# sdwyc/ROLO

Hardware: AMD Instinct MI355X
Metric: scans/sec (128k-pt frame, 20 GN iters) (higher is better)
Workload: dtype f64

## Files before the change

### rolo_amd/csrc/knn_cov.hip

```cpp
#include <cstdio>
#include <cstring>
#include <string.h>
#include "rolo_internal.hpp"
#include "dev_math.hpp"
#include "voxel_dev.hpp"
#ifdef ROLO_KNN_ROCPRIM_SORT
#include <rocprim/rocprim.hpp>
#endif
#include <cfloat>
#include <climits>

namespace rolo {

namespace {


constexpr int BBOX_BLOCKS = 128;
constexpr int BBOX_PART = 16;

__global__ __launch_bounds__(256) void bbox_kernel(KnnPair A, int* bbox) {
  __shared__ float smn[4][3], smx[4][3];
  const int which = blockIdx.x / BBOX_BLOCKS, blk = blockIdx.x - which * BBOX_BLOCKS;
  const float4* __restrict__ p = A.c[which].xyz;
  const int n = A.c[which].n;
// ... 477 lines not shown
#pragma unroll
    for (int i = 0; i < 9; i++) Ci[i] /= nrm;
    inv3(Ci, out);
  } else {
    const double A[9] = {cxx, cxy, cxz, cxy, cyy, cyz, cxz, cyz, czz};
    double U[9], V[9], sv[3];
    jacobi_svd3(A, U, sv, V);
    double v0 = 1, v1 = 1, v2 = 1e-3;
    if (reg == ROLO_REG_MIN_EIG) { v0 = fmax(sv[0], 1e-3); v1 = fmax(sv[1], 1e-3); v2 = fmax(sv[2], 1e-3); }
    else if (reg == ROLO_REG_NORMALIZED_MIN_EIG) { double m = fmax(sv[0], fmax(sv[1], sv[2])); v0 = fmax(sv[0] / m, 1e-3); v1 = fmax(sv[1] / m, 1e-3); v2 = fmax(sv[2] / m, 1e-3); }
    else if (reg == ROLO_REG_PLANE_S) { double s = sv[0] + sv[1] + sv[2]; v0 = sv[0] / s; v1 = sv[1] / s; v2 = 1e-3; }
#pragma unroll
    for (int a = 0; a < 3; a++)
#pragma unroll
      for (int b = 0; b < 3; b++) out[a * 3 + b] = (U[a * 3 + 0] * v0) * V[b * 3 + 0] + (U[a * 3 + 1] * v1) * V[b * 3 + 1] + (U[a * 3 + 2] * v2) * V[b * 3 + 2];
    if (nrm && reg == ROLO_REG_PLANE) {
      const double s3 = U[0 * 3 + 2] * V[0 * 3 + 2] + U[1 * 3 + 2] * V[1 * 3 + 2] + U[2 * 3 + 2] * V[2 * 3 + 2];
      const double al = sqrt(1.0 - (s3 < 0 ? -1e-3 : 1e-3));
      const double s1 = U[0 * 3 + 0] * V[0 * 3 + 0] + U[1 * 3 + 0] * V[1 * 3 + 0] + U[2 * 3 + 0] * V[2 * 3 + 0];
      const double s2 = U[0 * 3 + 1] * V[0 * 3 + 1] + U[1 * 3 + 1] * V[1 * 3 + 1] + U[2 * 3 + 1] * V[2 * 3 + 1];
      const bool plane_form = s1 > 0 && s2 > 0;
      const size_t pn = (size_t)n;
      nrm[qi] = plane_form ? al * V[0 * 3 + 2] : __builtin_nan(""); nrm[pn + qi] = al * V[1 * 3 + 2]; nrm[2 * pn + qi] = al * V[2 * 3 + 2];
    }
  }
  const size_t pitch = (size_t)n;
  c6[0] = out[0]; c6[1] = 0.5 * (out[1] + out[3]); c6[2] = 0.5 * (out[2] + out[6]); c6[3] = out[4]; c6[4] = 0.5 * (out[5] + out[7]); c6[5] = out[8];
#pragma unroll
  for (int d = 0; d < 6; d++) cov[d * pitch + qi] = c6[d];
}

template <int KMAX>
ROLO_DEV void knn_neighbourhood_moments(const int (&ki)[KMAX], int kk, const float4* __restrict__ orig, double (&m6)[6]) {
  float px[KMAX], py[KMAX], pz[KMAX];
#pragma unroll
  for (int u = 0; u < KMAX; u++) {
    const float4 p = (u < kk) ? orig[ki[u]] : make_float4(0.f, 0.f, 0.f, 0.f);
    px[u] = p.x; py[u] = p.y; pz[u] = p.z;
  }
  double mx = 0, my = 0, mz = 0;
#pragma unroll
  for (int u = 0; u < KMAX; u++) if (u < kk) { mx += (double)px[u]; my += (double)py[u]; mz += (double)pz[u]; }
  mx /= kk; my /= kk; mz /= kk;
  double cxx = 0, cxy = 0, cxz = 0, cyy = 0, cyz = 0, czz = 0;
#pragma unroll
  for (int u = 0; u < KMAX; u++) if (u < kk) {
    const double ax = (double)px[u] - mx, ay = (double)py[u] - my, az = (double)pz[u] - mz;
    cxx += ax * ax; cxy += ax * ay; cxz += ax * az; cyy += ay * ay; cyz += ay * az; czz += az * az;
  }
  m6[0] = cxx / kk; m6[1] = cxy / kk; m6[2] = cxz / kk; m6[3] = cyy / kk; m6[4] = cyz / kk; m6[5] = czz / kk;
}

template <int KMAX>
ROLO_DEV void knn_covariance_tail(const int (&ki)[KMAX], int kk, const float4* __restrict__ orig, int n, int qi, int reg,
                                  double* __restrict__ cov, double (&c6)[6], double* __restrict__ nrm = nullptr) {
  double m6[6];
  knn_neighbourhood_moments<KMAX>(ki, kk, orig, m6);
  knn_covariance_finish(m6[0], m6[1], m6[2], m6[3], m6[4], m6[5], n, qi, reg, cov, c6, nrm);
}

ROLO_DEV void knn_covariance_tail_loop(const int32_t* __restrict__ nbr, size_t n_sorted, int j, int kk, const float4* __restrict__ orig, int n, int qi, int reg,
                                       double* __restrict__ cov, double (&c6)[6], double* __restrict__ nrm = nullptr) {
  double mx = 0, my = 0, mz = 0;
  for (int u = 0; u < kk; u++) { const float4 p = orig[nbr[(size_t)u * n_sorted + j]]; mx += (double)p.x; my += (double)p.y; mz += (double)p.z; }
  mx /= kk; my /= kk; mz /= kk;
  double cxx = 0, cxy = 0, cxz = 0, cyy = 0, cyz = 0, czz = 0;
  for (int u = 0; u < kk; u++) {
    const float4 p = orig[nbr[(size_t)u * n_sorted + j]];
    const double ax = (double)p.x - mx, ay = (double)p.y - my, az = (double)p.z - mz;
    cxx += ax * ax; cxy += ax * ay; cxz += ax * az; cyy += ay * ay; cyz += ay * az; czz += az * az;
  }
  cxx /= kk; cxy /= kk; cxz /= kk; cyy /= kk; cyz /= kk; czz /= kk;
  knn_covariance_finish(cxx, cxy, cxz, cyy, cyz, czz, n, qi, reg, cov, c6, nrm);
}
}
}

#include "knn_walk.hpp"

namespace rolo {

bool knn_voxel_fuse_supported() {
#ifdef ROLO_KNN_ROCPRIM_SORT
  return false;
#else
  return true;
#endif
}

size_t knn_bbox_ints() { return BBOX_PART + 2 * BBOX_BLOCKS * 6; }

size_t knn_sort_temp_bytes(int n) {
#ifdef ROLO_KNN_ROCPRIM_SORT
  size_t bytes = 0;
  (void)rocprim::radix_sort_pairs(nullptr, bytes, (uint32_t*)nullptr, (uint32_t*)nullptr, (uint32_t*)nullptr, (uint32_t*)nullptr,
                                  (size_t)n, 0, 31, (hipStream_t)0);
  return bytes;
#else
  (void)n;
  return sizeof(int) * SORT_PASSES * SORT_NB * SORT_D;
#endif
}

hipError_t launch_knn_build(const KnnPair& A_in, void* sort_tmp, size_t sort_tmp_bytes, uint32_t* keys0, uint32_t* keys1,
                            uint32_t* vals0, uint32_t* vals1, int* bbox, const VoxelFuse& vf, hipStream_t s) {
  KnnPair A = A_in;
  bool have_parts = true;
  for (int i = 0; i < A.n_clouds; i++) have_parts = have_parts && A.c[i].bpart != nullptr && A.c[i].n_bpart > 0;
  if (!have_parts) for (int i = 0; i < A.n_clouds; i++) { A.c[i].bpart = bbox + BBOX_PART + i * BBOX_BLOCKS * 6; A.c[i].n_bpart = BBOX_BLOCKS; }
  const int nc = A.n_clouds;
  const int n_total = A.c[0].n + (nc > 1 ? A.c[1].n : 0);
#ifdef ROLO_KNN_ROCPRIM_SORT
  const int tile_ = ((n_total + SORT_NB - 1) / SORT_NB + SORT_T - 1) / SORT_T * SORT_T;
  if (!have_parts) bbox_kernel<<<BBOX_BLOCKS * nc, 256, 0, s>>>(A, bbox);
  morton_kernel<<<SORT_NB + (vf.enabled ? VF_CLEAR_BLOCKS : 0), SORT_T, 0, s>>>(A, bbox, keys0, vals0, n_total, tile_, nullptr, vf);
  hipError_t e = rocprim::radix_sort_pairs(sort_tmp, sort_tmp_bytes, keys0, keys1, vals0, vals1, (size_t)n_total, 0, nc > 1 ? KEY_BITS : KEY_BITS - 1, s);
  if (e != hipSuccess) return e;
  const uint32_t* order = vals1;
#else
  (void)sort_tmp_bytes;
  int* cnt = static_cast<int*>(sort_tmp);
  const int gvf = vf.enabled ? ((vf.n_tgt + SORT_PASSES - 1) / SORT_PASSES + SORT_T - 1) / SORT_T : 0;
  const int tile = ((n_total + SORT_NB - 1) / SORT_NB + SORT_T - 1) / SORT_T * SORT_T;
  if (!have_parts) bbox_kernel<<<BBOX_BLOCKS * nc, 256, 0, s>>>(A, bbox);
  morton_kernel<<<SORT_NB + (vf.enabled ? VF_CLEAR_BLOCKS : 0), SORT_T, 0, s>>>(A, bbox, keys0, vals0, n_total, tile, cnt, vf);
  uint32_t *ki = keys0, *vi = vals0, *ko = keys1, *vo = vals1;
  for (int p = 0; p < SORT_PASSES; p++) {
    if (p > 0) sort_hist_kernel<<<SORT_NB, SORT_T, 0, s>>>(ki, n_total, tile, p, cnt);
    sort_scatter_kernel<<<SORT_NB + gvf, SORT_T, 0, s>>>(ki, vi, ko, vo, n_total, tile, p, cnt, vf);
    uint32_t* t1 = ki; ki = ko; ko = t1; t1 = vi; vi = vo; vo = t1;
  }
  const uint32_t* order = vi;
#endif
  static_assert(256 % KNN_LEAF == 0 && (KNN_LEAF & (KNN_LEAF - 1)) == 0, "leaf_kernel reduces a leaf inside a wavefront");
  const int l0 = (A.c[0].P * KNN_LEAF + 255) / 256, l1 = nc > 1 ? (A.c[1].P * KNN_LEAF + 255) / 256 : 0;
  leaf_kernel<<<l0 + l1, 256, 0, s>>>(A, l0, order);
  constexpr int LPB = 256 / KNN_LEAF;
  int count0 = A.c[0].P >= LPB ? A.c[0].P / LPB : A.c[0].P, count1 = nc > 1 ? (A.c[1].P >= LPB ? A.c[1].P / LPB : A.c[1].P) : 1;
  while (count0 > 1 || count1 > 1) {
    const int chunk0 = count0 < 512 ? count0 : 512, chunk1 = count1 < 512 ? count1 : 512;
    const int b0 = count0 > 1 ? count0 / chunk0 : 0, b1 = count1 > 1 ? count1 / chunk1 : 0;
    tree_reduce_kernel<<<b0 + b1, 256, 0, s>>>(A.c[0].boxes, count0, chunk0, b0, nc > 1 ? A.c[1].boxes : nullptr, count1, chunk1);
    if (count0 > 1) count0 /= chunk0;
    if (count1 > 1) count1 /= chunk1;
  }
  return hipGetLastError();
}

#ifdef ROLO_KNN_STATS
extern "C" int rolo_debug_wave_records(unsigned* out ) {
  (void)hipDeviceSynchronize();
  return hipMemcpyFromSymbol(out, HIP_SYMBOL(g_knn_wave_rec), sizeof(unsigned) * 16384 * 8) == hipSuccess ? 0 : -1;
}
#endif

static inline int slice_blocks(const KnnCloud& c) { return (c.q_end - c.q_begin + 255) / 256; }

constexpr int KNN_SUB_MAX_PACKETS = 1792;
hipError_t launch_knn_walk(const KnnPair& A, int k, int regularization_or_minus1, const VoxelFuse& vf, hipStream_t s, int coop_budget, int* lanes_out, bool device_busy, bool moments) {
  if (lanes_out) *lanes_out = 1;
  constexpr int QPB = 256;
  const int n0 = A.c[0].q_end - A.c[0].q_begin, n1 = A.n_clouds > 1 ? A.c[1].q_end - A.c[1].q_begin : 0;
  const int g0 = (n0 + QPB - 1) / QPB, g1 = (n1 + QPB - 1) / QPB;
  if (g0 + g1 == 0) return hipSuccess;
  (void)vf;
  constexpr int pad = 0;
  if (k > 64) {
    if (regularization_or_minus1 >= 0) return hipErrorInvalidValue;
    KnnPair R = A;
    for (int r = 0; 64 * r < k; r++) {
      const int kr = k - 64 * r < 64 ? k - 64 * r : 64;
      for (int i = 0; i < R.n_clouds; i++) { R.c[i].slot0 = 64 * r; R.c[i].k_total = k; }
      if (r == 0) knn_walk_kernel<64, false><<<g0 + g1, 256, pad, s>>>(R, g0, kr, -1);
      else knn_walk_kernel<64, false, true><<<g0 + g1, 256, pad, s>>>(R, g0, kr, -1);
    }
    return hipGetLastError();
  }
  if (k == 20) {
    if (regularization_or_minus1 >= 0) knn_walk_kernel<20, true><<<g0 + g1, 256, pad, s>>>(A, g0, k, regularization_or_minus1);
    else if (coop_budget > 0) {
      const int packets = (n0 + 63) / 64 + (n1 + 63) / 64;
      static const int force_nw = [] {
        const char* e = getenv("ROLO_KNN_COOP_NW");
        if (!e) return 0;
        const int v = atoi(e);
        if (v == 4 || v == 8 || v == 16) return v;
        fprintf(stderr, "librolo_hip: ROLO_KNN_COOP_NW=%s is not one of 4 / 8 / 16: ignored\n", e);
        return 0;
      }();
      const int nw = force_nw ? force_nw : (packets >= 16 * 256 ? 16 : (packets >= 8 * 256 ? 8 : 4));
      const int G4 = g0 + g1, G = (G4 + nw / 4 - 1) / (nw / 4);
      if (nw == 16) knn_walk_coop_kernel<16><<<G, 1024, 0, s>>>(A, g0, G4, coop_budget);
      else if (nw == 8) knn_walk_coop_kernel<8><<<G, 512, 0, s>>>(A, g0, G4, coop_budget);
      else knn_walk_coop_kernel<4><<<G, 256, 0, s>>>(A, g0, G4, coop_budget);
    }
    else {
      static const int sub_env = [] {
        const char* e = getenv("ROLO_KNN_SUB");
        if (!e) return -1;
        const int v = atoi(e);
        if (v == 0 || v == 1 || v == 2 || v == 4) return v;
        fprintf(stderr, "librolo_hip: ROLO_KNN_SUB=%s is not one of 0 / 1 / 2 / 4: ignored (the walk is picked by size)\n", e);
        return -1;
      }();
      const int packets = (n0 + 63) / 64 + (n1 + 63) / 64;
      const int lanes = sub_env < 0 ? (packets <= KNN_SUB_MAX_PACKETS ? 4 : (device_busy ? 0 : 2)) : (sub_env == 2 ? 2 : (sub_env ? 4 : 0));
      if (lanes_out) *lanes_out = lanes ? lanes : 1;
      static const int walk_pad = [] {
        const char* e = getenv("ROLO_KNN_WALK_WGS"); const int v = e ? atoi(e) : 0;
        const int pad_bytes = (v >= 1 && v <= 8) ? (160 * 1024 / v - 1024 - 512) & ~255 : 0;
        if (pad_bytes > 48 * 1024) {
          bool ok = hipFuncSetAttribute(reinterpret_cast<const void*>(&knn_walk_kernel<20, false>), hipFuncAttributeMaxDynamicSharedMemorySize, pad_bytes) == hipSuccess;
          ok = ok && hipFuncSetAttribute(reinterpret_cast<const void*>(&knn_walk_sub_kernel<2>), hipFuncAttributeMaxDynamicSharedMemorySize, pad_bytes) == hipSuccess;
          ok = ok && hipFuncSetAttribute(reinterpret_cast<const void*>(&knn_walk_sub_kernel<4>), hipFuncAttributeMaxDynamicSharedMemorySize, pad_bytes) == hipSuccess;
          if (!ok) { (void)hipGetLastError(); fprintf(stderr, "librolo_hip: ROLO_KNN_WALK_WGS=%d needs %d bytes of dynamic LDS, which this runtime refuses: ignored\n", v, pad_bytes); return 0; }
        }
        return pad_bytes;
      }();
      if (lanes == 4) { const int s0 = (n0 + 63) / 64, s1 = (n1 + 63) / 64; if (moments) knn_walk_sub_kernel<4, true><<<s0 + s1, 256, walk_pad, s>>>(A, s0); else knn_walk_sub_kernel<4><<<s0 + s1, 256, walk_pad, s>>>(A, s0); }
      else if (lanes == 2) { const int s0 = (n0 + 127) / 128, s1 = (n1 + 127) / 128; if (moments) knn_walk_sub_kernel<2, true><<<s0 + s1, 256, walk_pad, s>>>(A, s0); else knn_walk_sub_kernel<2><<<s0 + s1, 256, walk_pad, s>>>(A, s0); }
      else if (moments) knn_walk_kernel<20, false, false, true><<<g0 + g1, 256, walk_pad, s>>>(A, g0, k, -1);
      else knn_walk_kernel<20, false><<<g0 + g1, 256, walk_pad, s>>>(A, g0, k, -1);
    }
  }
  else {
    if (k > 32) {
      if (regularization_or_minus1 >= 0) knn_walk_kernel<64, true><<<g0 + g1, 256, pad, s>>>(A, g0, k, regularization_or_minus1);
      else knn_walk_kernel<64, false><<<g0 + g1, 256, pad, s>>>(A, g0, k, -1);
    } else if (regularization_or_minus1 >= 0) knn_walk_kernel<32, true><<<g0 + g1, 256, pad, s>>>(A, g0, k, regularization_or_minus1);
    else knn_walk_kernel<32, false><<<g0 + g1, 256, pad, s>>>(A, g0, k, -1);
  }
  return hipGetLastError();
}

hipError_t launch_knn_unstage(const KnnPair& A, bool own_slice_only, const VoxelFuse& vf, hipStream_t s) {
  const int g0 = own_slice_only ? slice_blocks(A.c[0]) : (A.c[0].n_sorted + 255) / 256;
  const int g1 = A.n_clouds > 1 ? (own_slice_only ? slice_blocks(A.c[1]) : (A.c[1].n_sorted + 255) / 256) : 0;
  if (g0 + g1 == 0) return hipSuccess;
  VoxelFuse v = vf;
  if (own_slice_only) v.enabled = 0;
  knn_unstage_kernel<<<g0 + g1, 256, 0, s>>>(A, g0, own_slice_only ? 1 : 0, v);
  return hipGetLastError();
}

hipError_t launch_knn_tail(const KnnPair& A, int k, int regularization, const VoxelFuse& vf, hipStream_t s, bool moments) {
  const int g0 = slice_blocks(A.c[0]), g1 = A.n_clouds > 1 ? slice_blocks(A.c[1]) : 0;
  if (g0 + g1 == 0) return hipSuccess;
  if (k > 64) knn_tail_loop_kernel<<<g0 + g1, 256, 0, s>>>(A, g0, k, regularization, vf);
  else if (k == 20 && moments) knn_tail_kernel<20, true><<<g0 + g1, 256, 0, s>>>(A, g0, k, regularization, vf);
  else if (k == 20) knn_tail_kernel<20><<<g0 + g1, 256, 0, s>>>(A, g0, k, regularization, vf);
  else if (k <= 32) knn_tail_kernel<32><<<g0 + g1, 256, 0, s>>>(A, g0, k, regularization, vf);
  else knn_tail_kernel<64><<<g0 + g1, 256, 0, s>>>(A, g0, k, regularization, vf);
  return hipGetLastError();
}

}
```

### rolo_amd/csrc/knn_packet.hpp

```cpp
#pragma once
#include "rolo_internal.hpp"
#include "dev_math.hpp"
#include <cfloat>
#include <climits>

#ifndef KNN_STAT
#ifdef ROLO_KNN_STATS
#define KNN_STAT(x) x
#else
#define KNN_STAT(x)
#endif
#endif

namespace rolo {
namespace {

constexpr int WALK_STACK = KNN_WALK_STACK;

ROLO_DEV float box_d2(const float4& lo, const float4& hi, const float4& q) {
  float dx = fmaxf(fmaxf(__fsub_rn(lo.x, q.x), __fsub_rn(q.x, hi.x)), 0.f);
  float dy = fmaxf(fmaxf(__fsub_rn(lo.y, q.y), __fsub_rn(q.y, hi.y)), 0.f);
  float dz = fmaxf(fmaxf(__fsub_rn(lo.z, q.z), __fsub_rn(q.z, hi.z)), 0.f);
  return __fadd_rn(__fadd_rn(__fmul_rn(dx, dx), __fmul_rn(dy, dy)), __fmul_rn(dz, dz));
}

ROLO_DEV double key_pack(float d2, int idx) {
  return __longlong_as_double((long long)(((unsigned long long)__float_as_uint(d2) << 32) | (unsigned)idx));
}
ROLO_DEV float key_d2(double k) { return __uint_as_float((unsigned)((unsigned long long)__double_as_longlong(k) >> 32)); }
ROLO_DEV int key_idx(double k) { return (int)(unsigned)((unsigned long long)__double_as_longlong(k) & 0xffffffffull); }

ROLO_DEV double vmin_f64(double a, double b) { double r; asm("v_min_f64 %0, %1, %2" : "=v"(r) : "v"(a), "v"(b)); return r; }
ROLO_DEV double vmax_f64(double a, double b) { double r; asm("v_max_f64 %0, %1, %2" : "=v"(r) : "v"(a), "v"(b)); return r; }
#ifndef ROLO_KNN_SPLIT_MINMAX
ROLO_DEV void insert_slot(double& ks, double ksm1, double c) { asm("v_min_f64 %0, %1, %0\n\tv_max_f64 %0, %2, %0" : "+&v"(ks) : "v"(c), "v"(ksm1)); }
#else
ROLO_DEV void insert_slot(double& ks, double ksm1, double c) { ks = vmax_f64(ksm1, vmin_f64(c, ks)); }
#endif
#ifndef ROLO_KNN_B1
#define ROLO_KNN_B1 15
#define ROLO_KNN_B2 10
#define ROLO_KNN_B3 5
#endif
template <int KMAX>
ROLO_DEV void insert_tiered(double (&K)[KMAX], double ck) {
  constexpr int B1 = KMAX == 20 ? ROLO_KNN_B1 : 3 * (KMAX / 4), B2 = KMAX == 20 ? ROLO_KNN_B2 : 2 * (KMAX / 4), B3 = KMAX == 20 ? ROLO_KNN_B3 : KMAX / 4;
#pragma unroll
  for (int s = KMAX - 1; s >= B1; s--) insert_slot(K[s], K[s - 1], ck);
  if (__any(ck < K[B1 - 1])) {
#pragma unroll
    for (int s = B1 - 1; s >= B2; s--) insert_slot(K[s], K[s - 1], ck);
    if (__any(ck < K[B2 - 1])) {
#pragma unroll
      for (int s = B2 - 1; s >= B3; s--) insert_slot(K[s], K[s - 1], ck);
      if (__any(ck < K[B3 - 1])) {
#pragma unroll
        for (int s = B3 - 1; s >= 1; s--) insert_slot(K[s], K[s - 1], ck);
        K[0] = vmin_f64(ck, K[0]);
      }
    }
  }
}

typedef float sgpr16 __attribute__((ext_vector_type(16)));
#ifndef ROLO_KNN_ASM_LOADS
#define ROLO_KNN_ASM_LOADS 0
#endif
constexpr bool KNN_PLAIN_ASM = ROLO_KNN_ASM_LOADS != 0;
ROLO_DEV const float4* uniform_ptr(const float4* p) {
  const unsigned long long v = (unsigned long long)p;
  const unsigned lo = (unsigned)__builtin_amdgcn_readfirstlane((int)(unsigned)v), hi = (unsigned)__builtin_amdgcn_readfirstlane((int)(unsigned)(v >> 32));
  return (const float4*)(((unsigned long long)hi << 32) | lo);
}
template <bool ASM>
ROLO_DEV void sload_leaf(const float4* __restrict__ p_, float4 (&pts)[KNN_LEAF]) {
  if (!ASM) {
#pragma unroll
    for (int u = 0; u < KNN_LEAF; u++) pts[u] = p_[u];
    return;
  }
  const float4* p = uniform_ptr(p_);
#if 1
  static_assert(KNN_LEAF == 16 || KNN_LEAF == 8, "leaf size");
  sgpr16 a, b;
  if (KNN_LEAF == 16) {
    sgpr16 c, d;
    asm("s_load_dwordx16 %0, %4, 0x0\n\ts_load_dwordx16 %1, %4, 0x40\n\ts_load_dwordx16 %2, %4, 0x80\n\ts_load_dwordx16 %3, %4, 0xc0\n\ts_waitcnt lgkmcnt(0)"
        : "=&s"(a), "=&s"(b), "=&s"(c), "=&s"(d) : "s"(p));
#pragma unroll
    for (int u = 0; u < 4; u++) { pts[8 + u] = make_float4(c[4 * u], c[4 * u + 1], c[4 * u + 2], c[4 * u + 3]); pts[12 + u] = make_float4(d[4 * u], d[4 * u + 1], d[4 * u + 2], d[4 * u + 3]); }
  } else {
    asm("s_load_dwordx16 %0, %2, 0x0\n\ts_load_dwordx16 %1, %2, 0x40\n\ts_waitcnt lgkmcnt(0)" : "=&s"(a), "=&s"(b) : "s"(p));
  }
#pragma unroll
  for (int u = 0; u < 4; u++) { pts[u] = make_float4(a[4 * u], a[4 * u + 1], a[4 * u + 2], a[4 * u + 3]); pts[4 + u] = make_float4(b[4 * u], b[4 * u + 1], b[4 * u + 2], b[4 * u + 3]); }
#else
#pragma unroll
  for (int u = 0; u < KNN_LEAF; u++) pts[u] = p[u];
#endif
}
template <bool ASM>
ROLO_DEV void sload_node(const float4* __restrict__ p_, float4& llo, float4& lhi, float4& rlo, float4& rhi) {
  if (!ASM) { llo = p_[0]; lhi = p_[1]; rlo = p_[2]; rhi = p_[3]; return; }
  const float4* p = uniform_ptr(p_);
#if 1
  sgpr16 a;
  asm("s_load_dwordx16 %0, %1, 0x0\n\ts_waitcnt lgkmcnt(0)" : "=s"(a) : "s"(p));
  llo = make_float4(a[0], a[1], a[2], a[3]); lhi = make_float4(a[4], a[5], a[6], a[7]); rlo = make_float4(a[8], a[9], a[10], a[11]); rhi = make_float4(a[12], a[13], a[14], a[15]);
#else
  llo = p[0]; lhi = p[1]; rlo = p[2]; rhi = p[3];
#endif
}

template <int KMAX, bool LOWER = false, bool CAP = false, bool ASM = false>
ROLO_DEV void knn_score_leaf(const float4* __restrict__ sorted, int g, const float4& q, double (&K)[KMAX], int kk, double& bkey, float& bd,
                             unsigned& n_ins, unsigned& lane_acc, unsigned& rounds, double lo = 0.0, double bcap = 0.0) {
  float4 pts[KNN_LEAF];
  sload_leaf<ASM>(sorted + KNN_LEAF * (size_t)g, pts);
  KNN_STAT(const double bkey0 = bkey; unsigned my_acc = 0;)
#ifdef ROLO_KNN_STATS2
  unsigned my_cur = 0;
#endif
#pragma unroll
  for (int u = 0; u < KNN_LEAF; u++) {
    const float4 c = pts[u];
    const float dx = q.x - c.x, dy = q.y - c.y, dz = q.z - c.z;
    const float cd = ((dx * dx) + (dy * dy)) + (dz * dz);
    const double ck0 = key_pack(cd, __float_as_int(c.w));
    const double ck = (LOWER && !(ck0 > lo)) ? key_pack(INFINITY, INT_MAX) : ck0;
    KNN_STAT(if (__any(ck < bkey)) { n_ins++; lane_acc += (unsigned)__popcll(__ballot(ck < bkey)); })
    KNN_STAT(if (ck < bkey0) my_acc++;)
#ifdef ROLO_KNN_STATS2
    if (ck < bkey) my_cur++;
#endif
    if (ck < bkey) {
      insert_tiered<KMAX>(K, ck);
#pragma unroll
      for (int s = 0; s < KMAX; s++) if (s == kk - 1) bkey = K[s];
      if (CAP) bkey = vmin_f64(bkey, bcap);
      bd = key_d2(bkey);
    }
  }
#ifdef ROLO_KNN_STATS
#ifdef ROLO_KNN_STATS2
  rounds += my_cur;
  (void)my_acc;
#else
  { unsigned m = my_acc;
    for (int off = 32; off > 0; off >>= 1) m = max(m, (unsigned)__shfl_xor((int)m, off, 64));
    rounds += m; }
#endif
#endif
}

template <int CTRL>
ROLO_DEV double dpp_f64(double x) {
  const long long v = __double_as_longlong(x);
  const int lo = __builtin_amdgcn_mov_dpp((int)(unsigned)(unsigned long long)v, CTRL, 0xF, 0xF, true);
  const int hi = __builtin_amdgcn_mov_dpp((int)(unsigned)((unsigned long long)v >> 32), CTRL, 0xF, 0xF, true);
  return __longlong_as_double((long long)(((unsigned long long)(unsigned)hi << 32) | (unsigned)lo));
}
template <int ST> ROLO_DEV double sub_xchg(double x) { return ST == 0 ? dpp_f64<0xB1>(x) : ST == 1 ? dpp_f64<0x4E>(x) : dpp_f64<0x141>(x); }
template <int SUB> ROLO_DEV double sub_min(double x) {
  x = vmin_f64(x, sub_xchg<0>(x));
  if (SUB >= 4) x = vmin_f64(x, sub_xchg<1>(x));
  if (SUB >= 8) x = vmin_f64(x, sub_xchg<2>(x));
  return x;
}
template <int SUB> ROLO_DEV double sub_max(double x) {
  x = vmax_f64(x, sub_xchg<0>(x));
  if (SUB >= 4) x = vmax_f64(x, sub_xchg<1>(x));
  if (SUB >= 8) x = vmax_f64(x, sub_xchg<2>(x));
  return x;
}

ROLO_DEV int xcd_contiguous_block(int b, int G, int wpb = 4) {
#ifdef ROLO_KNN_NO_XCD_REMAP
  return b;
#else
  if (G * wpb <= 2048) {
    const int x = b & 7, k = b >> 3, q = G >> 3, r = G & 7;
    return x * q + min(x, r) + k;
  }
  const int RUN = 256 / wpb, GROUP = 8 * RUN;
  if (b >= G / GROUP * GROUP) return b;
  const int grp = b / GROUP, o = b - grp * GROUP;
  return grp * GROUP + (o & 7) * RUN + (o >> 3);
#endif
}

typedef __attribute__((address_space(3))) int lds_int;
typedef __attribute__((address_space(3))) double lds_double;
constexpr int COOP_RING = 16;
struct CoopPub { lds_int* ring; lds_int* head; lds_int* tail; lds_double* cap; int budget; };

template <int KMAX, bool LOWER, bool CAP, bool PUBLISH, bool ASM>
ROLO_DEV void packet_walk(const float4* __restrict__ sorted, const float4* __restrict__ boxes, int P, int g_own0, int g_own1, const float4& q, double (&K)[KMAX], int kk,
                          double& bkey, float& bd, double lo, double bcap, lds_int* stk, int& sp, int h, const CoopPub& pub, int& n_scored, int& n_published,
                          unsigned& st_nodes, unsigned& st_leaves, unsigned& st_ins, unsigned& st_lane, unsigned& st_rounds, unsigned& st_push) {
  (void)st_push; (void)pub; (void)n_scored; (void)n_published;
  while (true) {
    h = __builtin_amdgcn_readfirstlane(h);
    if (h < P) {
      st_nodes++;
      float4 llo, lhi, rlo, rhi;
      sload_node<ASM>(boxes + 4 * (size_t)h, llo, lhi, rlo, rhi);
      const float bl = box_d2(llo, lhi, q), br = box_d2(rlo, rhi, q);
      const bool okl = (bl <= bd) && (bl < INFINITY), okr = (br <= bd) && (br < INFINITY);
      const unsigned long long ml = __ballot(okl), mr = __ballot(okr);
      if (ml != 0ull && mr != 0ull) {
        const unsigned long long pref = __ballot((okl || okr) && (bl <= br));
        const bool left_first = 2 * __popcll(pref) >= __popcll(ml | mr);
        if (sp < WALK_STACK) { stk[sp] = left_first ? 2 * h + 1 : 2 * h; sp++; KNN_STAT(st_push++;) }
        h = left_first ? 2 * h : 2 * h + 1;
        continue;
      }
      if (ml != 0ull) { h = 2 * h; continue; }
      if (mr != 0ull) { h = 2 * h + 1; continue; }
    } else {
      const int g = h - P;
      if (g < g_own0 || g >= g_own1) {
        knn_score_leaf<KMAX, LOWER, CAP, ASM>(sorted, g, q, K, kk, bkey, bd, st_ins, st_lane, st_rounds, lo, bcap);
        st_leaves++;
        if (PUBLISH) n_scored++;
      }
    }
    if (sp == 0) return;
    if (PUBLISH && n_scored >= pub.budget && sp >= 2) {
      const int lane = threadIdx.x & 63;
      const int hd = __builtin_amdgcn_readfirstlane(*pub.head);
      const int tl = __builtin_amdgcn_readfirstlane(__hip_atomic_load((int*)pub.tail, __ATOMIC_RELAXED, __HIP_MEMORY_SCOPE_WORKGROUP));
      if (hd == tl) {
        const int m = min(sp >> 1, 4);
        if (lane < m) pub.ring[(hd + lane) % COOP_RING] = stk[lane];
        pub.cap[lane] = bkey;
        const int keep = sp - m;
        const int e = lane < keep ? stk[m + lane] : 0;
        if (lane < keep) stk[lane] = e;
        sp = keep;
        __builtin_amdgcn_fence(__ATOMIC_RELEASE, "workgroup");
        if (lane == 0) __hip_atomic_store((int*)pub.head, hd + m, __ATOMIC_RELAXED, __HIP_MEMORY_SCOPE_WORKGROUP);
        n_published += m;
      }
    }
    sp--;
    h = stk[sp];
  }
}

ROLO_DEV int coop_steal(lds_int* ring, lds_int* head, lds_int* tail) {
  int e = -1;
  if ((threadIdx.x & 63) == 0) {
    while (true) {
      const int t = __hip_atomic_load((int*)tail, __ATOMIC_RELAXED, __HIP_MEMORY_SCOPE_WORKGROUP);
      const int hd = __hip_atomic_load((int*)head, __ATOMIC_RELAXED, __HIP_MEMORY_SCOPE_WORKGROUP);
      if (t >= hd) break;
      __builtin_amdgcn_fence(__ATOMIC_ACQUIRE, "workgroup");
      const int v = ring[t % COOP_RING];
      int expect = t;
      if (__hip_atomic_compare_exchange_strong((int*)tail, &expect, t + 1, __ATOMIC_RELAXED, __ATOMIC_RELAXED, __HIP_MEMORY_SCOPE_WORKGROUP)) { e = v; break; }
    }
  }
  return __builtin_amdgcn_readfirstlane(e);
}

}
}
```

### rolo_amd/csrc/knn_walk.hpp

```cpp
#pragma once
#ifdef ROLO_KNN_STATS
#define KNN_STAT(x) x
#else
#define KNN_STAT(x)
#endif
#include "knn_packet.hpp"

namespace rolo {
namespace {

ROLO_DEV double* stage_area(const KnnCloud& cl, unsigned add) {
  double* s = cl.stage;
  if (cl.stage_epoch) {
    const unsigned long long e = __hip_atomic_load(cl.stage_epoch, __ATOMIC_RELAXED, __HIP_MEMORY_SCOPE_SYSTEM) + add;
    if (e & 1ull) s += cl.stage_alt;
  }
  return s;
}

#ifdef ROLO_KNN_STATS
__device__ unsigned g_knn_wave_rec[16384][8];
#endif

template <int KMAX>
ROLO_DEV void walk_write_lists(const KnnCloud& cl, const double (&K)[KMAX], int kk, double bkey, int qi, int j) {
  int ki[KMAX];
#pragma unroll
  for (int u = 0; u < KMAX; u++) ki[u] = key_idx(K[u]);
  const int slot0 = (KMAX == 64) ? cl.slot0 : 0;
  const int ktot = (KMAX == 64 && cl.k_total) ? cl.k_total : kk;
  if (cl.knn_idx) {
#pragma unroll
    for (int u = 0; u < KMAX; u++) if (u < kk) { cl.knn_idx[(size_t)qi * ktot + slot0 + u] = ki[u]; cl.knn_d2[(size_t)qi * ktot + slot0 + u] = key_d2(K[u]); }
  }
  if (KMAX == 64 && cl.lower) cl.lower[j] = bkey;
  int32_t* __restrict__ nbr = cl.nbr;
#pragma unroll
  for (int u = 0; u < KMAX; u++) nbr[(size_t)(slot0 + u) * cl.n_sorted + j] = ki[u];
}

template <int KMAX>
ROLO_DEV void walk_write_moments(const KnnCloud& cl, const double (&K)[KMAX], int kk, int qi, int j, int (*s_ki)[256]) {
  if (cl.knn_idx) {
#pragma unroll
    for (int u = 0; u < KMAX; u++) if (u < kk) { cl.knn_idx[(size_t)qi * kk + u] = key_idx(K[u]); cl.knn_d2[(size_t)qi * kk + u] = key_d2(K[u]); }
  }
  const int tid = threadIdx.x;
#pragma unroll
  for (int u = 0; u < KMAX; u++) s_ki[u][tid] = key_idx(K[u]);
  const float4* __restrict__ orig = cl.xyz;
  double mx = 0, my = 0, mz = 0;
#pragma unroll 5
  for (int u = 0; u < kk; u++) { const float4 p = orig[s_ki[u][tid]]; mx += (double)p.x; my += (double)p.y; mz += (double)p.z; }
  mx /= kk; my /= kk; mz /= kk;
  double cxx = 0, cxy = 0, cxz = 0, cyy = 0, cyz = 0, czz = 0;
#pragma unroll 5
  for (int u = 0; u < kk; u++) {
    const float4 p = orig[s_ki[u][tid]];
    const double ax = (double)p.x - mx, ay = (double)p.y - my, az = (double)p.z - mz;
    cxx += ax * ax; cxy += ax * ay; cxz += ax * az; cyy += ay * ay; cyz += ay * az; czz += az * az;
  }
  double* __restrict__ mom = reinterpret_cast<double*>(cl.nbr);
  const size_t pitch = (size_t)cl.n_sorted;
  mom[j] = cxx / kk; mom[pitch + j] = cxy / kk; mom[2 * pitch + j] = cxz / kk; mom[3 * pitch + j] = cyy / kk; mom[4 * pitch + j] = cyz / kk; mom[5 * pitch + j] = czz / kk;
}

#ifndef ROLO_KNN_WALK_OCC
#define ROLO_KNN_WALK_OCC 4
#endif
#ifndef ROLO_KNN_PACKET
#define ROLO_KNN_PACKET 64
#endif
#ifndef ROLO_KNN_SEED_EXTRA
#define ROLO_KNN_SEED_EXTRA 1
#endif
static_assert(ROLO_KNN_PACKET == 64, "one query per lane");

template <int KMAX, bool LOWER, bool ASM>
ROLO_DEV void walk_seeds(const float4* __restrict__ sorted, int g_mine0, int g_own0, int g_own1, int n_leaves, const float4& q, double (&K)[KMAX], int kk, double& bkey, float& bd, double lo,
                         unsigned& st_leaves, unsigned& st_ins, unsigned& st_lane, unsigned& st_rounds) {
  const int n_own = min(g_mine0 + 64 / KNN_LEAF, n_leaves) - g_mine0, n_before = g_mine0 - g_own0;
  for (int i = 0; i < g_own1 - g_own0; i++) {
    const int g = i < n_own ? g_mine0 + i : (i - n_own < n_before ? g_own0 + (i - n_own) : g_mine0 + (i - n_before));
    knn_score_leaf<KMAX, LOWER, false, ASM>(sorted, g, q, K, kk, bkey, bd, st_ins, st_lane, st_rounds, lo);
    st_leaves++;
  }
}

template <int KMAX, bool FUSE_TAIL, bool LOWER = false, bool MOMENTS = false>
__global__ __launch_bounds__(256, KMAX > 32 ? 2 : (MOMENTS ? 6 : ROLO_KNN_WALK_OCC)) void knn_walk_kernel(KnnPair A, int split, int k, int reg) {
  __shared__ int stk[4][WALK_STACK];
  __shared__ int s_ki[MOMENTS ? KMAX : 1][256];
  const int tid = threadIdx.x;
  const int wv = tid >> 6;
  const int blk = xcd_contiguous_block((int)blockIdx.x, (int)gridDim.x, 4);
  const int which = blk >= split ? 1 : 0;
  const float4* __restrict__ sorted = A.c[which].sorted;
  const float4* __restrict__ boxes = A.c[which].boxes;
  const int n_sorted = A.c[which].n_sorted, P = A.c[which].P;
  const int lane_ = tid & 63;
  const int j = A.c[which].q_begin + (blk - (which ? split : 0)) * 256 + wv * 64 + lane_;
  float4 q = make_float4(0.f, 0.f, 0.f, 0.f);
  int qi = INT_MAX;
  if (j < A.c[which].q_end) { q = sorted[j]; qi = __float_as_int(q.w); }
  const bool active = qi != INT_MAX;
  const int kk = (KMAX == 20) ? 20 : k;
  const int n_leaves = n_sorted / KNN_LEAF;
  unsigned st_nodes = 0, st_leaves = 0, st_ins = 0, st_lane = 0, st_rounds = 0, st_push = 0;

  const double sentinel = key_pack(INFINITY, INT_MAX);
  double K[KMAX];
#pragma unroll
  for (int u = 0; u < KMAX; u++) K[u] = sentinel;
  float bd = active ? INFINITY : -1.0f;
  double bkey = active ? sentinel : key_pack(0.f, 0);

  const int g_mine0 = __builtin_amdgcn_readfirstlane(j / KNN_LEAF);
  const int g_own0 = max(g_mine0 - ROLO_KNN_SEED_EXTRA, 0);
  const int g_own1 = min(g_mine0 + 64 / KNN_LEAF + ROLO_KNN_SEED_EXTRA, n_leaves);
  double lo = 0.0;
  if (LOWER && active) lo = A.c[which].lower[j];
  (void)lo;
  walk_seeds<KMAX, LOWER, KNN_PLAIN_ASM>(sorted, g_mine0, g_own0, g_own1, n_leaves, q, K, kk, bkey, bd, lo, st_leaves, st_ins, st_lane, st_rounds);

  int sp = 0;
  int h = 1;
#ifdef ROLO_KNN_STATS
  unsigned long long wt0;
  asm("s_memrealtime %0\n\ts_waitcnt lgkmcnt(0)\n\ts_mov_b32 %1, 1" : "=s"(wt0), "=s"(h));
#endif
  { const CoopPub none{}; int n_scored = 0, n_pub = 0;
    packet_walk<KMAX, LOWER, false, false, KNN_PLAIN_ASM>(sorted, boxes, P, g_own0, g_own1, q, K, kk, bkey, bd, lo, 0.0, (lds_int*)&stk[wv][0], sp, h, none, n_scored, n_pub, st_nodes, st_leaves, st_ins, st_lane, st_rounds, st_push); }
#ifdef ROLO_KNN_STATS
  { unsigned long long wt1; asm volatile("s_memrealtime %0\n\ts_waitcnt lgkmcnt(0)" : "=s"(wt1));
    unsigned st_rounds_rec = st_rounds;
#ifdef ROLO_KNN_STATS2
    for (int off = 32; off > 0; off >>= 1) st_rounds_rec = max(st_rounds_rec, (unsigned)__shfl_xor((int)st_rounds_rec, off, 64));
#endif
    const unsigned wid = blockIdx.x * 4 + (threadIdx.x >> 6);
    if ((threadIdx.x & 63) == 0 && wid < 16384) {
      g_knn_wave_rec[wid][0] = st_nodes; g_knn_wave_rec[wid][1] = st_leaves; g_knn_wave_rec[wid][2] = st_ins; g_knn_wave_rec[wid][3] = st_push;
      g_knn_wave_rec[wid][4] = (unsigned)wt0; g_knn_wave_rec[wid][5] = (unsigned)wt1; g_knn_wave_rec[wid][6] = st_lane; g_knn_wave_rec[wid][7] = st_rounds_rec;
    } }
#endif
  (void)st_nodes; (void)st_leaves; (void)st_ins; (void)st_lane; (void)st_rounds; (void)st_push;

  if (!active) return;

  if (MOMENTS) {
    walk_write_moments<KMAX>(A.c[which], K, kk, qi, j, s_ki);
    return;
  }
  if (!FUSE_TAIL) {
    walk_write_lists<KMAX>(A.c[which], K, kk, bkey, qi, j);
    return;
  }
  const KnnCloud& cl = A.c[which];
  int ki[KMAX];
#pragma unroll
  for (int u = 0; u < KMAX; u++) ki[u] = key_idx(K[u]);
  if (cl.knn_idx) {
#pragma unroll
    for (int u = 0; u < KMAX; u++) if (u < kk) { cl.knn_idx[(size_t)qi * kk + u] = ki[u]; cl.knn_d2[(size_t)qi * kk + u] = key_d2(K[u]); }
  }
  if (cl.stage) {
    double* o = stage_area(cl, 1) + (size_t)(j / cl.chunk) * cl.seg + cl.stage_off + (size_t)(j % cl.chunk) * 6;
    double c6[6]; knn_covariance_tail<KMAX>(ki, kk, cl.xyz, 1, 0, reg, o, c6);
  } else {
    double c6[6]; knn_covariance_tail<KMAX>(ki, kk, cl.xyz, cl.n, qi, reg, cl.cov, c6, cl.nrm);
  }
}

template <int ST> ROLO_DEV void merge20(double (&K)[20]) {
#pragma unroll
  for (int j = 0; j < 10; j++) {
    const double o1 = sub_xchg<ST>(K[19 - j]), o2 = sub_xchg<ST>(K[j]);
    K[j] = vmin_f64(K[j], o1);
    K[19 - j] = vmin_f64(K[19 - j], o2);
  }
#pragma unroll
  for (int d = 16; d >= 1; d >>= 1) {
#pragma unroll
    for (int p = 12; p < 32; p++) {
      if ((p & d) == 0) {
        const int x = p - 12, y = p + d - 12;
        const double lo = vmin_f64(K[x], K[y]);
        K[y] = vmax_f64(K[x], K[y]);
        K[x] = lo;
      }
    }
  }
}

#ifdef ROLO_KNN_WALK_MAXOCC
#define ROLO_KNN_WALK_OCC_ATTR __attribute__((amdgpu_waves_per_eu(ROLO_KNN_WALK_MAXOCC, ROLO_KNN_WALK_MAXOCC)))
#else
#define ROLO_KNN_WALK_OCC_ATTR
#endif
template <int SUB, bool MOMENTS = false>
__global__ __launch_bounds__(256, MOMENTS ? 6 : ROLO_KNN_WALK_OCC) ROLO_KNN_WALK_OCC_ATTR void knn_walk_sub_kernel(KnnPair A, int split ) {
  constexpr int SH = SUB == 2 ? 1 : 2, QPW = 64 / SUB, PPL = KNN_LEAF / SUB, KMAX = 20, E = 4 / SUB , OWN = QPW / KNN_LEAF;
  static_assert(SUB == 2 || SUB == 4, "lanes per query");
  static_assert(KNN_LEAF == 16, "a wavefront's queries are whole leaves");
  __shared__ int stk_[4][WALK_STACK];
  __shared__ int s_ki[MOMENTS ? KMAX : 1][256];
  const int tid = threadIdx.x;
  const int wv = __builtin_amdgcn_readfirstlane(tid >> 6), lane = tid & 63, sub = lane & (SUB - 1), ql = lane >> SH;
  const int blk = xcd_contiguous_block((int)blockIdx.x, (int)gridDim.x, 4);
  const int which = blk >= split ? 1 : 0;
  const KnnCloud& cl = A.c[which];
  const float4* __restrict__ sorted = cl.sorted;
  const float4* __restrict__ boxes = cl.boxes;
  const int n_sorted = cl.n_sorted, P = cl.P, n_leaves = n_sorted / KNN_LEAF;
  const int j0 = cl.q_begin + ((blk - (which ? split : 0)) * 4 + wv) * QPW;
  const int j = j0 + ql;
  float4 q = make_float4(0.f, 0.f, 0.f, 0.f);
  int qi = INT_MAX;
  if (j < cl.q_end) { q = sorted[j]; qi = __float_as_int(q.w); }
  const bool active = qi != INT_MAX;
  const double sentinel = key_pack(INFINITY, INT_MAX);
  double K[KMAX];
#pragma unroll
  for (int u = 0; u < KMAX; u++) K[u] = sentinel;
  double B = active ? sentinel : key_pack(0.f, 0);
  float bd = active ? INFINITY : -1.0f;
  auto score = [&](int g) {
    const float4* __restrict__ leaf = sorted + KNN_LEAF * (size_t)g;
    bool changed = false;
#pragma unroll
    for (int t0 = 0; t0 < PPL; t0 += 4) {
      float4 c[4];
#pragma unroll
      for (int t = 0; t < 4; t++) c[t] = leaf[(t0 + t) * SUB + sub];
#pragma unroll
      for (int t = 0; t < 4; t++) {
        const float dx = q.x - c[t].x, dy = q.y - c[t].y, dz = q.z - c[t].z;
        const float cd = ((dx * dx) + (dy * dy)) + (dz * dz);
        const double ck = key_pack(cd, __float_as_int(c[t].w));
        if (ck < B) { insert_tiered<KMAX>(K, ck); changed = true; }
      }
    }
    if (__any(changed)) {
      B = vmin_f64(vmin_f64(B, sub_min<SUB>(K[KMAX - 1])), sub_max<SUB>(K[KMAX / SUB - 1]));
      bd = key_d2(B);
    }
  };
  const int g_mine = min(j0 / KNN_LEAF, n_leaves - 1);
  const int g_own0 = max(g_mine - ROLO_KNN_SEED_EXTRA, 0), g_own1 = min(g_mine + OWN + ROLO_KNN_SEED_EXTRA, n_leaves);
  for (int g = g_mine; g < min(g_mine + OWN, n_leaves); g++) score(g);
  for (int g = g_own0; g < g_own1; g++) if (g < g_mine || g >= g_mine + OWN) score(g);
  {
    lds_int* stk = (lds_int*)&stk_[wv][0];
    int sp = 0, h = 1;
    while (true) {
      h = __builtin_amdgcn_readfirstlane(h);
      if (2 * h < P) {
        float d[E]; bool ok[E];
        float dm = INFINITY;
#pragma unroll
        for (int e = 0; e < E; e++) {
          const int c = sub * E + e;
          const float4 blo = boxes[8 * (size_t)h + 2 * c], bhi = boxes[8 * (size_t)h + 2 * c + 1];
          d[e] = box_d2(blo, bhi, q);
          ok[e] = (d[e] <= bd) && (d[e] < INFINITY);
          dm = fminf(dm, ok[e] ? d[e] : INFINITY);
        }
        dm = fminf(dm, __int_as_float(__builtin_amdgcn_mov_dpp(__float_as_int(dm), 0xB1, 0xF, 0xF, true)));
        if (SUB == 4) dm = fminf(dm, __int_as_float(__builtin_amdgcn_mov_dpp(__float_as_int(dm), 0x4E, 0xF, 0xF, true)));
        unsigned long long m[E], v[E];
#pragma unroll
        for (int e = 0; e < E; e++) { m[e] = __ballot(ok[e]); v[e] = __ballot(ok[e] && d[e] == dm); }
        int key[4];
#pragma unroll
        for (int c = 0; c < 4; c++) {
          const unsigned long long sel = (SUB == 4 ? 0x1111111111111111ull : 0x5555555555555555ull) << (c / E);
          key[c] = (m[c % E] & sel) != 0ull ? __popcll(v[c % E] & sel) * 4 + (3 - c) : -1;
        }
        auto cx = [](int& a, int& bb) { const int hi = max(a, bb), lo = min(a, bb); a = hi; bb = lo; };
        cx(key[0], key[1]); cx(key[2], key[3]); cx(key[0], key[2]); cx(key[1], key[3]); cx(key[1], key[2]);
        if (key[0] >= 0) {
#pragma unroll
          for (int r = 3; r >= 1; r--) if (key[r] >= 0 && sp < WALK_STACK) { stk[sp] = 4 * h + (3 - (key[r] & 3)); sp++; }
          h = 4 * h + (3 - (key[0] & 3));
          continue;
        }
      } else if (h < P) {
        const int c = sub & 1;
        const float4 blo = boxes[4 * (size_t)h + 2 * c], bhi = boxes[4 * (size_t)h + 2 * c + 1];
        const float d = box_d2(blo, bhi, q);
        const float o = __int_as_float(__builtin_amdgcn_mov_dpp(__float_as_int(d), 0xB1, 0xF, 0xF, true));
        const bool ok = (d <= bd) && (d < INFINITY), oko = (o <= bd) && (o < INFINITY);
        const unsigned long long m = __ballot(ok);
        const unsigned long long ml = m & 0x5555555555555555ull, mr = m & 0xaaaaaaaaaaaaaaaaull;
        if (ml != 0ull && mr != 0ull) {
          const unsigned long long pref = __ballot(c == 0 && (ok || oko) && (d <= o));
          const unsigned long long either = (ml | (mr >> 1)) & 0x5555555555555555ull;
          const bool left_first = 2 * __popcll(pref) >= __popcll(either);
          if (sp < WALK_STACK) { stk[sp] = left_first ? 2 * h + 1 : 2 * h; sp++; }
          h = left_first ? 2 * h : 2 * h + 1;
          continue;
        }
        if (ml != 0ull) { h = 2 * h; continue; }
        if (mr != 0ull) { h = 2 * h + 1; continue; }
      } else {
        const int g = h - P;
        if (g < g_own0 || g >= g_own1) score(g);
      }
      if (sp == 0) break;
      sp--;
      h = stk[sp];
    }
  }
  merge20<0>(K);
  if (SUB == 4) merge20<1>(K);
  if (MOMENTS) {
    if (active && sub == 0) walk_write_moments<KMAX>(cl, K, KMAX, qi, j, s_ki);
    return;
  }
  constexpr int NS = KMAX / SUB;
  int ki[NS];
#pragma unroll
  for (int t = 0; t < NS; t++) {
    if (SUB == 4) {
      const double k01 = sub & 1 ? K[NS + t] : K[t], k23 = sub & 1 ? K[3 * NS + t] : K[2 * NS + t];
      ki[t] = key_idx(sub & 2 ? k23 : k01);
    } else {
      ki[t] = key_idx(sub & 1 ? K[NS + t] : K[t]);
    }
  }
  if (!active) return;
  int32_t* __restrict__ nbr = cl.nbr;
#pragma unroll
  for (int t = 0; t < NS; t++) nbr[(size_t)(sub * NS + t) * n_sorted + j] = ki[t];
  if (cl.knn_idx && sub == 0) {
#pragma unroll
    for (int u = 0; u < KMAX; u++) { cl.knn_idx[(size_t)qi * KMAX + u] = key_idx(K[u]); cl.knn_d2[(size_t)qi * KMAX + u] = key_d2(K[u]); }
  }
}

template <int NW> struct CoopCfg { static constexpr int NSLOT = NW == 16 ? 14 : (NW == 8 ? 7 : 3); };

template <int NW>
__global__ __launch_bounds__(64 * NW, ROLO_KNN_WALK_OCC) void knn_walk_coop_kernel(KnnPair A, int split4 , int G4 , int budget) {
  constexpr int KMAX = 20, kk = 20, NSLOT = CoopCfg<NW>::NSLOT;
// ... 249 lines not shown
```

Baseline: 4247.

## Seed KNN lists with sorting networks and bitonic merges instead of per-key insertion

Seed-leaf scoring now builds each query's top-20 list differently. The first leaf's 16 keys are loaded and ordered with a sorting network. Each following seed leaf is split into chunks of 8 keys, each chunk is sorted, and it is merged into the list with a bitonic merge. This replaces divergent tiered insertion, with its per-key __any branches, by branch-free min/max networks. The price is a fixed amount of min/max work even when few keys qualify. The change also adds per-tier insertion counters under the stats build and factors out the shared bitonic helper.

```diff
diff --git a/rolo_amd/csrc/knn_cov.hip b/rolo_amd/csrc/knn_cov.hip
--- a/rolo_amd/csrc/knn_cov.hip
+++ b/rolo_amd/csrc/knn_cov.hip
@@ -653,6 +653,10 @@
   (void)hipDeviceSynchronize();
   return hipMemcpyFromSymbol(out, HIP_SYMBOL(g_knn_wave_rec), sizeof(unsigned) * 16384 * 8) == hipSuccess ? 0 : -1;
 }
+extern "C" int rolo_debug_wave_records2(unsigned* out ) {
+  (void)hipDeviceSynchronize();
+  return hipMemcpyFromSymbol(out, HIP_SYMBOL(g_knn_wave_rec2), sizeof(unsigned) * 16384 * 8) == hipSuccess ? 0 : -1;
+}
 #endif
 
 static inline int slice_blocks(const KnnCloud& c) { return (c.q_end - c.q_begin + 255) / 256; }
diff --git a/rolo_amd/csrc/knn_packet.hpp b/rolo_amd/csrc/knn_packet.hpp
--- a/rolo_amd/csrc/knn_packet.hpp
+++ b/rolo_amd/csrc/knn_packet.hpp
@@ -42,9 +42,12 @@
 #define ROLO_KNN_B2 10
 #define ROLO_KNN_B3 5
 #endif
+template <int KMAX> struct InsertTiers {
+  static constexpr int B1 = KMAX == 20 ? ROLO_KNN_B1 : 3 * (KMAX / 4), B2 = KMAX == 20 ? ROLO_KNN_B2 : 2 * (KMAX / 4), B3 = KMAX == 20 ? ROLO_KNN_B3 : KMAX / 4;
+};
 template <int KMAX>
 ROLO_DEV void insert_tiered(double (&K)[KMAX], double ck) {
-  constexpr int B1 = KMAX == 20 ? ROLO_KNN_B1 : 3 * (KMAX / 4), B2 = KMAX == 20 ? ROLO_KNN_B2 : 2 * (KMAX / 4), B3 = KMAX == 20 ? ROLO_KNN_B3 : KMAX / 4;
+  constexpr int B1 = InsertTiers<KMAX>::B1, B2 = InsertTiers<KMAX>::B2, B3 = InsertTiers<KMAX>::B3;
 #pragma unroll
   for (int s = KMAX - 1; s >= B1; s--) insert_slot(K[s], K[s - 1], ck);
   if (__any(ck < K[B1 - 1])) {
@@ -60,6 +63,39 @@
       }
     }
   }
+}
+
+ROLO_DEV void cmpx(double& a, double& b) {
+  double lo, hi;
+  asm("v_min_f64 %0, %2, %3\n\tv_max_f64 %1, %2, %3" : "=&v"(lo), "=v"(hi) : "v"(a), "v"(b));
+  a = lo; b = hi;
+}
+template <int N, int M>
+ROLO_DEV void sort_net(double (&a)[M]) {
+  static_assert(N <= M && (N & (N - 1)) == 0, "a power of two of the array's slots");
+#pragma unroll
+  for (int p = 1; p < N; p <<= 1)
+#pragma unroll
+    for (int k = p; k >= 1; k >>= 1)
+#pragma unroll
+      for (int j = k % p; j + k < N; j += 2 * k)
+#pragma unroll
+        for (int i = 0; i < k; i++)
+          if ((i + j) / (2 * p) == (i + j + k) / (2 * p)) cmpx(a[i + j], a[i + j + k]);
+}
+ROLO_DEV void bitonic_sort20(double (&K)[20]) {
+#pragma unroll
+  for (int d = 16; d >= 1; d >>= 1) {
+#pragma unroll
+    for (int p = 12; p < 32; p++)
+      if ((p & d) == 0) cmpx(K[p - 12], K[p + d - 12]);
+  }
+}
+template <int C>
+ROLO_DEV void merge_sorted20(double (&K)[20], const double (&S)[C]) {
+#pragma unroll
+  for (int i = 20 - C; i < 20; i++) K[i] = vmin_f64(K[i], S[19 - i]);
+  bitonic_sort20(K);
 }
 
 typedef float sgpr16 __attribute__((ext_vector_type(16)));
@@ -112,9 +148,18 @@
 #endif
 }
 
+template <bool LOWER>
+ROLO_DEV double leaf_key(const float4& q, const float4& c, double lo) {
+  const float dx = q.x - c.x, dy = q.y - c.y, dz = q.z - c.z;
+  const float cd = ((dx * dx) + (dy * dy)) + (dz * dz);
+  const double ck0 = key_pack(cd, __float_as_int(c.w));
+  return (LOWER && !(ck0 > lo)) ? key_pack(INFINITY, INT_MAX) : ck0;
+}
+
 template <int KMAX, bool LOWER = false, bool CAP = false, bool ASM = false>
 ROLO_DEV void knn_score_leaf(const float4* __restrict__ sorted, int g, const float4& q, double (&K)[KMAX], int kk, double& bkey, float& bd,
-                             unsigned& n_ins, unsigned& lane_acc, unsigned& rounds, double lo = 0.0, double bcap = 0.0) {
+                             unsigned& n_ins, unsigned& lane_acc, unsigned& rounds, double lo = 0.0, double bcap = 0.0, unsigned* st_tier = nullptr) {
+  (void)st_tier;
   float4 pts[KNN_LEAF];
   sload_leaf<ASM>(sorted + KNN_LEAF * (size_t)g, pts);
   KNN_STAT(const double bkey0 = bkey; unsigned my_acc = 0;)
@@ -123,12 +168,10 @@
 #endif
 #pragma unroll
   for (int u = 0; u < KNN_LEAF; u++) {
-    const float4 c = pts[u];
-    const float dx = q.x - c.x, dy = q.y - c.y, dz = q.z - c.z;
-    const float cd = ((dx * dx) + (dy * dy)) + (dz * dz);
-    const double ck0 = key_pack(cd, __float_as_int(c.w));
-    const double ck = (LOWER && !(ck0 > lo)) ? key_pack(INFINITY, INT_MAX) : ck0;
+    const double ck = leaf_key<LOWER>(q, pts[u], lo);
     KNN_STAT(if (__any(ck < bkey)) { n_ins++; lane_acc += (unsigned)__popcll(__ballot(ck < bkey)); })
+    KNN_STAT(if (st_tier) { using T = InsertTiers<KMAX>;
+               st_tier[0] += __any(ck < bkey && ck < K[T::B1 - 1]); st_tier[1] += __any(ck < bkey && ck < K[T::B2 - 1]); st_tier[2] += __any(ck < bkey && ck < K[T::B3 - 1]); })
     KNN_STAT(if (ck < bkey0) my_acc++;)
 #ifdef ROLO_KNN_STATS2
     if (ck < bkey) my_cur++;
@@ -197,7 +240,7 @@
 template <int KMAX, bool LOWER, bool CAP, bool PUBLISH, bool ASM>
 ROLO_DEV void packet_walk(const float4* __restrict__ sorted, const float4* __restrict__ boxes, int P, int g_own0, int g_own1, const float4& q, double (&K)[KMAX], int kk,
                           double& bkey, float& bd, double lo, double bcap, lds_int* stk, int& sp, int h, const CoopPub& pub, int& n_scored, int& n_published,
-                          unsigned& st_nodes, unsigned& st_leaves, unsigned& st_ins, unsigned& st_lane, unsigned& st_rounds, unsigned& st_push) {
+                          unsigned& st_nodes, unsigned& st_leaves, unsigned& st_ins, unsigned& st_lane, unsigned& st_rounds, unsigned& st_push, unsigned* st_tier = nullptr) {
   (void)st_push; (void)pub; (void)n_scored; (void)n_published;
   while (true) {
     h = __builtin_amdgcn_readfirstlane(h);
@@ -220,7 +263,7 @@
     } else {
       const int g = h - P;
       if (g < g_own0 || g >= g_own1) {
-        knn_score_leaf<KMAX, LOWER, CAP, ASM>(sorted, g, q, K, kk, bkey, bd, st_ins, st_lane, st_rounds, lo, bcap);
+        knn_score_leaf<KMAX, LOWER, CAP, ASM>(sorted, g, q, K, kk, bkey, bd, st_ins, st_lane, st_rounds, lo, bcap, st_tier);
         st_leaves++;
         if (PUBLISH) n_scored++;
       }
diff --git a/rolo_amd/csrc/knn_walk.hpp b/rolo_amd/csrc/knn_walk.hpp
--- a/rolo_amd/csrc/knn_walk.hpp
+++ b/rolo_amd/csrc/knn_walk.hpp
@@ -20,6 +20,7 @@
 
 #ifdef ROLO_KNN_STATS
 __device__ unsigned g_knn_wave_rec[16384][8];
+__device__ unsigned g_knn_wave_rec2[16384][8];
 #endif
 
 template <int KMAX>
@@ -76,13 +77,46 @@
 #endif
 static_assert(ROLO_KNN_PACKET == 64, "one query per lane");
 
+#ifndef ROLO_KNN_SEED_MERGE
+#define ROLO_KNN_SEED_MERGE 1
+#endif
+
 template <int KMAX, bool LOWER, bool ASM>
 ROLO_DEV void walk_seeds(const float4* __restrict__ sorted, int g_mine0, int g_own0, int g_own1, int n_leaves, const float4& q, double (&K)[KMAX], int kk, double& bkey, float& bd, double lo,
-                         unsigned& st_leaves, unsigned& st_ins, unsigned& st_lane, unsigned& st_rounds) {
+                         unsigned& st_leaves, unsigned& st_ins, unsigned& st_lane, unsigned& st_rounds, unsigned* st_tier = nullptr) {
   const int n_own = min(g_mine0 + 64 / KNN_LEAF, n_leaves) - g_mine0, n_before = g_mine0 - g_own0;
-  for (int i = 0; i < g_own1 - g_own0; i++) {
-    const int g = i < n_own ? g_mine0 + i : (i - n_own < n_before ? g_own0 + (i - n_own) : g_mine0 + (i - n_before));
-    knn_score_leaf<KMAX, LOWER, false, ASM>(sorted, g, q, K, kk, bkey, bd, st_ins, st_lane, st_rounds, lo);
+  const int n_seed = g_own1 - g_own0;
+  auto leaf = [&](int i) { return i < n_own ? g_mine0 + i : (i - n_own < n_before ? g_own0 + (i - n_own) : g_mine0 + (i - n_before)); };
+  if constexpr (KMAX == 20 && ROLO_KNN_SEED_MERGE != 0) {
+    static_assert(KNN_LEAF == 16, "a leaf is one list's first 16 keys, or two chunks of 8");
+    (void)kk;
+    if (n_seed <= 0) return;
+    {
+      float4 pts[KNN_LEAF];
+      sload_leaf<ASM>(sorted + KNN_LEAF * (size_t)leaf(0), pts);
+#pragma unroll
+      for (int u = 0; u < KNN_LEAF; u++) K[u] = vmin_f64(leaf_key<LOWER>(q, pts[u], lo), K[KMAX - 1]);
+      sort_net<KNN_LEAF>(K);
+    }
+    for (int i = 1; i < n_seed; i++) {
+      float4 pts[KNN_LEAF];
+      sload_leaf<ASM>(sorted + KNN_LEAF * (size_t)leaf(i), pts);
+#pragma unroll
+      for (int h = 0; h < KNN_LEAF; h += 8) {
+        double S[8];
+#pragma unroll
+        for (int u = 0; u < 8; u++) S[u] = leaf_key<LOWER>(q, pts[h + u], lo);
+        sort_net<8>(S);
+        merge_sorted20(K, S);
+        KNN_STAT(if (st_tier) st_tier[3]++;)
+      }
+    }
+    st_leaves += n_seed;
+    if (bd >= 0.f) { bkey = K[KMAX - 1]; bd = key_d2(bkey); }
+    return;
+  }
+  for (int i = 0; i < n_seed; i++) {
+    knn_score_leaf<KMAX, LOWER, false, ASM>(sorted, leaf(i), q, K, kk, bkey, bd, st_ins, st_lane, st_rounds, lo, 0.0, st_tier);
     st_leaves++;
   }
 }
@@ -121,7 +155,9 @@
   double lo = 0.0;
   if (LOWER && active) lo = A.c[which].lower[j];
   (void)lo;
-  walk_seeds<KMAX, LOWER, KNN_PLAIN_ASM>(sorted, g_mine0, g_own0, g_own1, n_leaves, q, K, kk, bkey, bd, lo, st_leaves, st_ins, st_lane, st_rounds);
+  unsigned st_tier[8] = {0, 0, 0, 0, 0, 0, 0, 0};
+  walk_seeds<KMAX, LOWER, KNN_PLAIN_ASM>(sorted, g_mine0, g_own0, g_own1, n_leaves, q, K, kk, bkey, bd, lo, st_leaves, st_ins, st_lane, st_rounds, st_tier);
+  KNN_STAT(const unsigned st_ins_seed = st_ins;)
 
   int sp = 0;
   int h = 1;
@@ -130,7 +166,8 @@
   asm("s_memrealtime %0\n\ts_waitcnt lgkmcnt(0)\n\ts_mov_b32 %1, 1" : "=s"(wt0), "=s"(h));
 #endif
   { const CoopPub none{}; int n_scored = 0, n_pub = 0;
-    packet_walk<KMAX, LOWER, false, false, KNN_PLAIN_ASM>(sorted, boxes, P, g_own0, g_own1, q, K, kk, bkey, bd, lo, 0.0, (lds_int*)&stk[wv][0], sp, h, none, n_scored, n_pub, st_nodes, st_leaves, st_ins, st_lane, st_rounds, st_push); }
+    packet_walk<KMAX, LOWER, false, false, KNN_PLAIN_ASM>(sorted, boxes, P, g_own0, g_own1, q, K, kk, bkey, bd, lo, 0.0, (lds_int*)&stk[wv][0], sp, h, none, n_scored, n_pub, st_nodes, st_leaves, st_ins, st_lane, st_rounds, st_push,
+                                                          st_tier + 4); }
 #ifdef ROLO_KNN_STATS
   { unsigned long long wt1; asm volatile("s_memrealtime %0\n\ts_waitcnt lgkmcnt(0)" : "=s"(wt1));
     unsigned st_rounds_rec = st_rounds;
@@ -141,9 +178,12 @@
     if ((threadIdx.x & 63) == 0 && wid < 16384) {
       g_knn_wave_rec[wid][0] = st_nodes; g_knn_wave_rec[wid][1] = st_leaves; g_knn_wave_rec[wid][2] = st_ins; g_knn_wave_rec[wid][3] = st_push;
       g_knn_wave_rec[wid][4] = (unsigned)wt0; g_knn_wave_rec[wid][5] = (unsigned)wt1; g_knn_wave_rec[wid][6] = st_lane; g_knn_wave_rec[wid][7] = st_rounds_rec;
+      g_knn_wave_rec2[wid][0] = st_ins_seed;
+#pragma unroll
+      for (int t = 0; t < 7; t++) g_knn_wave_rec2[wid][1 + t] = st_tier[t];
     } }
 #endif
-  (void)st_nodes; (void)st_leaves; (void)st_ins; (void)st_lane; (void)st_rounds; (void)st_push;
+  (void)st_nodes; (void)st_leaves; (void)st_ins; (void)st_lane; (void)st_rounds; (void)st_push; (void)st_tier;
 
   if (!active) return;
 
@@ -178,18 +218,7 @@
     K[j] = vmin_f64(K[j], o1);
     K[19 - j] = vmin_f64(K[19 - j], o2);
   }
-#pragma unroll
-  for (int d = 16; d >= 1; d >>= 1) {
-#pragma unroll
-    for (int p = 12; p < 32; p++) {
-      if ((p & d) == 0) {
-        const int x = p - 12, y = p + d - 12;
-        const double lo = vmin_f64(K[x], K[y]);
-        K[y] = vmax_f64(K[x], K[y]);
-        K[x] = lo;
-      }
-    }
-  }
+  bitonic_sort20(K);
 }
 
 #ifdef ROLO_KNN_WALK_MAXOCC
```

After: 4523 (median of 6 runs). 6.5% higher.
